# simonsobs/Pixell.jl

Measured on AMD Instinct MI355X. Metric: Mpix/s CAR bilinear reproject (Float64) + % HBM roofline, 1/2/4/8 MI355X, higher is better.
Workload: dtype f64

## Files before the change

### include/pixell_hip.h

```cpp
#ifndef PIXELL_HIP_H
#define PIXELL_HIP_H

#include <stddef.h>
#include <stdint.h>

#ifdef __cplusplus
extern "C" {
#endif

#define PXL_VERSION 100

typedef struct pxl_car_wcs {
    double cdelt[2];
    double crpix[2];
    double crval[2];
    double unit;
} pxl_car_wcs;

#define PXL_OK         0
#define PXL_EINVAL   (-22)
#define PXL_ENOMEM   (-12)
#define PXL_EHIP     (-5)
#define PXL_ENODEV   (-19)

// ... 40 lines not shown
                        double* ra, double* dec, void* stream);
int pxl_posmap_tan_f64(const pxl_car_wcs* wcs, const int64_t shape[2], int64_t row0, int64_t nrows,
                       double* ra, double* dec, void* stream);

typedef struct pxl_reproject_plan pxl_reproject_plan;

int pxl_reproject_plan_create(const pxl_car_wcs* wcs_in, const int64_t shape_in[3],
                              int64_t src_row0, int64_t src_nrows,
                              const pxl_car_wcs* wcs_out, const int64_t shape_out[2],
                              int64_t dst_row0, int64_t dst_nrows,
                              pxl_reproject_plan** plan);
int pxl_reproject_execute(pxl_reproject_plan* plan, const double* src, double* dst, void* stream);
int pxl_reproject_build_tables(pxl_reproject_plan* plan, void* stream);
int pxl_reproject_execute_rows(pxl_reproject_plan* plan, const double* src, double* dst,
                               int64_t r0, int64_t nr, void* stream);
int pxl_reproject_execute_f32(pxl_reproject_plan* plan, const float* src, float* dst, void* stream);
int pxl_reproject_execute_rows_f32(pxl_reproject_plan* plan, const float* src, float* dst,
                                   int64_t r0, int64_t nr, void* stream);
int pxl_reproject_plan_src_rows(const pxl_reproject_plan* plan, int64_t* lo, int64_t* hi);
int pxl_reproject_plan_rows_covered(const pxl_reproject_plan* plan, int64_t have_lo, int64_t have_hi,
                                    int64_t* lo, int64_t* hi);
int pxl_reproject_plan_set_variant(pxl_reproject_plan* plan, int variant);
int pxl_reproject_plan_destroy(pxl_reproject_plan* plan);

typedef struct pxl_halo_xfer {
    int32_t peer;
    int32_t reserved;
    int64_t row0;
    int64_t nrows;
} pxl_halo_xfer;
// ... 127 lines not shown
```

### pixell.jl_amd/_lib.py

```python
import ctypes as C
import os

_HERE = os.path.dirname(os.path.abspath(__file__))
LIB_PATH = os.environ.get("PXL_LIB_PATH", os.path.join(_HERE, "libpixell_hip.so"))

WRAP_NONE, WRAP_REWIND, WRAP_UNWIND = 0, 1, 2
FORM_RECIP, FORM_DIV, FORM_RECIP_AV = 0, 1, 2


class PixellHipError(RuntimeError):

    def __init__(self, code, message):
        super().__init__("libpixell_hip error %d: %s" % (code, message))
        self.code = code


class CarWCSStruct(C.Structure):
    _fields_ = [("cdelt", C.c_double * 2), ("crpix", C.c_double * 2), ("crval", C.c_double * 2),
                ("unit", C.c_double)]


_P = C.c_void_p
_I64 = C.c_int64
_WP = C.POINTER(CarWCSStruct)
# ... 10 lines not shown
    "pxl_pix2sky_car_soa_f64": (C.c_int, [_WP, _I64, _P, _P, _P, _P, C.c_int, _P]),
    "pxl_sky2pix_car_f64": (C.c_int, [_WP, _SHP, _I64, _P, _P, C.c_int, C.c_int, _P]),
    "pxl_sky2pix_car_soa_f64": (C.c_int, [_WP, _SHP, _I64, _P, _P, _P, _P, C.c_int, C.c_int, _P]),
    "pxl_posmap_car_f64": (C.c_int, [_WP, _SHP, _I64, _I64, _P, _P, C.c_int, _P]),
    "pxl_pixareamap_car_f64": (C.c_int, [_WP, _SHP, _I64, _I64, _P, _P]),
    "pxl_distance_transform_car_f64": (C.c_int, [_WP, _SHP, _P, _P, _P]),
    "pxl_sky2pix_tan_f64": (C.c_int, [_WP, _I64, _P, _P, _P, _P, _P]),
    "pxl_pix2sky_tan_f64": (C.c_int, [_WP, _I64, _P, _P, _P, _P, _P]),
    "pxl_posmap_tan_f64": (C.c_int, [_WP, _SHP, _I64, _I64, _P, _P, _P]),
    "pxl_reproject_plan_create": (C.c_int, [_WP, _SHP, _I64, _I64, _WP, _SHP, _I64, _I64, C.POINTER(_P)]),
    "pxl_reproject_execute": (C.c_int, [_P, _P, _P, _P]),
    "pxl_reproject_build_tables": (C.c_int, [_P, _P]),
    "pxl_reproject_execute_rows": (C.c_int, [_P, _P, _P, _I64, _I64, _P]),
    "pxl_reproject_execute_f32": (C.c_int, [_P, _P, _P, _P]),
    "pxl_reproject_execute_rows_f32": (C.c_int, [_P, _P, _P, _I64, _I64, _P]),
    "pxl_reproject_plan_src_rows": (C.c_int, [_P, C.POINTER(_I64), C.POINTER(_I64)]),
    "pxl_reproject_plan_rows_covered": (C.c_int, [_P, _I64, _I64, C.POINTER(_I64), C.POINTER(_I64)]),
    "pxl_reproject_plan_set_variant": (C.c_int, [_P, C.c_int]),
    "pxl_reproject_plan_destroy": (C.c_int, [_P]),
    "pxl_reproject_sharded_step_f64": (C.c_int, [_P, _P, _P, _I64, _I64, _P, C.c_int, _P, C.c_int, _P, _P]),
    "pxl_reproject_sharded_step_f32": (C.c_int, [_P, _P, _P, _I64, _I64, _P, C.c_int, _P, C.c_int, _P, _P]),
    "pxl_comm_unique_id": (C.c_int, [_P]),
    "pxl_comm_init_rank": (C.c_int, [_P, C.c_int, C.c_int, C.POINTER(_P)]),
    "pxl_comm_destroy": (C.c_int, [_P]),
    "pxl_comm_backend": (C.c_char_p, []),
    "pxl_reproject_car_bilinear_f64": (C.c_int, [_WP, _SHP, _P, _WP, _SHP, _P, _P]),
    "pxl_reproject_generic_bilinear_f64": (C.c_int, [_WP, C.c_int, _SHP, _P, _WP, C.c_int, _SHP, _P, _P]),
    "pxl_reproject_generic_last_tiles": (C.c_int, [C.POINTER(_I64), C.POINTER(_I64), _P]),
    "pxl_generic_plan_create": (C.c_int, [_WP, C.c_int, _SHP, _WP, C.c_int, _SHP, _P, C.POINTER(_P)]),
    "pxl_generic_plan_execute": (C.c_int, [_P, _I64, _P, _P, _P]),
# ... 89 lines not shown
```

### pixell.jl_amd/csrc/pxl_kernels.hip

```cpp
#include <hip/hip_runtime.h>

#include <algorithm>
#include <mutex>
#include <vector>
#include <cmath>
#include <cstdarg>
#include <cstdio>
#include <cstring>
#include <new>
#include <type_traits>

#include "pxl_device.h"

using namespace pxl;

static thread_local char g_err[512] = "";

static int fail(int code, const char* fmt, ...) {
    va_list ap;
    va_start(ap, fmt);
    vsnprintf(g_err, sizeof(g_err), fmt, ap);
    va_end(ap);
    return code;
}
// ... 72 lines not shown
static constexpr SlotRule kSlot32 = {256, 8.0, 4};
static int64_t seg_for(const SlotRule& r, int pairs, double sx) {
    double span = ceil((double)(r.cw * pairs) * sx) + r.slack;
    return ((int64_t)span + (r.align - 1)) & ~(r.align - 1);
}
static bool stageable(const SlotRule& r, int64_t sg, bool periodic, int64_t nx, double sy) {
    return (sg <= PXL_MAXCH * r.cw) && !(periodic && sg > nx) && sy <= 3.0;
}

struct pxl_reproject_plan {
    pxl_car_wcs win, wout;
    int64_t nx, ny, nc, src_row0, src_nrows;
    int64_t nxo, nyo, dst_row0, dst_nrows;
    int periodic;
    int device;
    Tables tab;
    void* table_mem;
    int32_t* h_yj0;
    int variant;
    int pairs;
    int pairs_dma;
    int seg_dma;
    int pairs_dma32;
    int seg_dma32;
    bool dma32_ok;
    int dypos;
    int rh;
    int rh32;
    int seg;
    int dxpos;
    int ns, pf;
    int nt;
    double* zero_page;
    bool staged_ok;
    bool vec_load;
    bool tables_built;
    hipStream_t comm_stream;
    hipEvent_t ev_ready, ev_halo;
    int64_t cov_have_lo, cov_have_hi, cov_lo, cov_hi;
};

struct DeviceState {
    hipMemPool_t pool;
    unsigned int* last_exact;
    int64_t generic_tiles;
};
static std::mutex g_dev_mu;
static DeviceState g_dev[64] = {};
static DeviceState* device_state() {
    int dev = 0;
    if (hipGetDevice(&dev) != hipSuccess || dev < 0 || dev >= 64) return nullptr;
// ... 171 lines not shown
    if (items < (int64_t)min_per_front * fronts) fronts = 1;
    int64_t per = (items + fronts - 1) / fronts;
    if (cap > 0 && per * fronts > cap) { fronts = 1; per = items; }
    return {fronts, per};
}

static int check_rows(const char* who, const int64_t shape[2], int64_t row0, int64_t nrows) {
    if (!shape || shape[0] < 1 || shape[1] < 1) return fail(PXL_EINVAL, "%s: bad shape", who);
    if (row0 < 0 || nrows < 0 || row0 + nrows > shape[1])
        return fail(PXL_EINVAL, "%s: rows [%lld, %lld) outside the map (ny=%lld)", who, (long long)row0,
                    (long long)(row0 + nrows), (long long)shape[1]);
    return PXL_OK;
}

template <class T>
static int reproject_rows_impl(pxl_reproject_plan* pl, const T* src, T* dst, int64_t r0, int64_t nr, void* stream) {
    if (!pl) return fail(PXL_EINVAL, "execute: null plan");
    if (r0 < 0 || nr < 0 || r0 + nr > pl->dst_nrows) return fail(PXL_EINVAL, "execute: rows outside the dst window");
    if (nr == 0) return PXL_OK;
    if (!dst || (!src && pl->src_nrows > 0)) return fail(PXL_EINVAL, "execute: null src/dst");
    if (!pl->tables_built) return fail(PXL_EINVAL, "execute_rows: tables not built");
    hipStream_t st = (hipStream_t)stream;
    constexpr bool f32 = std::is_same<T, float>::value;

    ReprojParams p;
    memset(&p, 0, sizeof(p));
    p.src = src; p.dst = dst;
    p.xi0 = pl->tab.xi0; p.xfx = pl->tab.xfx; p.yj0 = pl->tab.yj0; p.yfy = pl->tab.yfy;
    p.nx = pl->nx; p.ny = pl->ny; p.src_row0 = pl->src_row0; p.src_nrows = pl->src_nrows;
    p.nxo = pl->nxo; p.dst_row0 = pl->dst_row0; p.dst_nrows = pl->dst_nrows;
    p.r0 = r0; p.nr = nr; p.nc = (int32_t)pl->nc; p.periodic = pl->periodic;

    const bool aligned = (((uintptr_t)src & 15) == 0);
    bool staged = f32 ? (pl->dma32_ok && aligned) : pl->staged_ok;
    if (pl->variant == 1) staged = false;
    if (!staged) {
        int64_t work = ((pl->nxo + 1) / 2) * nr;
        dim3 g(stream_grid(work, 256), (unsigned)pl->nc);
        hipLaunchKernelGGL((k_reproject_gather<T>), g, dim3(256), 0, st, p);
        return check_launch("k_reproject_gather");
    }

    const bool vec = f32 ? true : (pl->vec_load && aligned);
    const bool use_dma = f32 ? true : (vec && pl->variant != 2);
    const int pairs = f32 ? pl->pairs_dma32 : (use_dma ? pl->pairs_dma : pl->pairs);
    const int cw = f32 ? kSlot32.cw : kSlot64.cw;
    const int TW = cw * pairs;
    p.seg = f32 ? pl->seg_dma32 : (use_dma ? pl->seg_dma : pl->seg);
    p.dxpos = pl->dxpos; p.dypos = pl->dypos;
    p.ntx = (int32_t)((pl->nxo + TW - 1) / TW);
    int rh = f32 ? pl->rh32 : pl->rh;
    while (rh > 4 && (int64_t)p.ntx * ((nr + rh - 1) / rh) * pl->nc < PXL_MIN_TILES) rh >>= 1;
    p.rh = rh;
    p.nty = (int32_t)((nr + rh - 1) / rh);
    p.ntiles = (int64_t)p.ntx * p.nty * pl->nc;
    p.tiles_per_xcd = (p.ntiles + 7) / 8;
    const int64_t nblocks = 8 * p.tiles_per_xcd;
    if (nblocks > 0x7fffffffLL) return fail(PXL_EINVAL, "execute: too many tiles (%lld)", (long long)nblocks);
    dim3 grid((unsigned)nblocks), block(64);
    if (use_dma) {
        const size_t esz = sizeof(T);
        p.ns = pl->ns; p.pf = pl->pf; p.zero_page = pl->zero_page;
        p.nt = pl->nt != 0;
        while ((size_t)p.ns * p.seg * esz > PXL_RING_BYTES && p.ns > 4) p.ns >>= 1;
        size_t dma_lds = (size_t)p.ns * (size_t)p.seg * esz;
        const int nch = (p.seg + cw - 1) / cw;
        return launch_reproject_dma_t<T>(pairs, nch, grid, dma_lds, st, p);
    }
    size_t lds_bytes = (size_t)PXL_NS * (size_t)pl->seg * sizeof(double);
// ... 48 lines not shown
        const ncclDataType_t dt = std::is_same<T, float>::value ? ncclFloat32 : ncclFloat64;
        ncclResult_t r = nc.GroupStart();
        for (int i = 0; i < nsends && r == ncclSuccess; ++i)
            for (int64_t c = 0; c < pl->nc && r == ncclSuccess; ++c)
                r = nc.Send((const char*)src + ((c * pl->src_nrows + (sends[i].row0 - lo)) * pl->nx) * esz,
                            (size_t)(sends[i].nrows * pl->nx), dt, sends[i].peer, (ncclComm_t)comm, pl->comm_stream);
        for (int i = 0; i < nrecvs && r == ncclSuccess; ++i)
            for (int64_t c = 0; c < pl->nc && r == ncclSuccess; ++c)
                r = nc.Recv((char*)src + ((c * pl->src_nrows + (recvs[i].row0 - lo)) * pl->nx) * esz,
                            (size_t)(recvs[i].nrows * pl->nx), dt, recvs[i].peer, (ncclComm_t)comm, pl->comm_stream);
        const ncclResult_t rend = nc.GroupEnd();
        if (r == ncclSuccess) r = rend;
        if (r != ncclSuccess) return fail(PXL_EHIP, "sharded_step: RCCL send/recv failed: %s", nc.GetErrorString(r));
        HIP_TRY(hipEventRecord(pl->ev_halo, pl->comm_stream));
    }
    rc = pxl_reproject_build_tables(pl, stream);
    if (rc) return rc;
    int64_t i_lo = 0, i_hi = pl->dst_nrows;
    if (exchange) {
        if (pl->cov_have_lo != own_row0 || pl->cov_have_hi != own_row0 + own_nrows || pl->cov_hi < pl->cov_lo) {
            rc = pxl_reproject_plan_rows_covered(pl, own_row0, own_row0 + own_nrows, &pl->cov_lo, &pl->cov_hi);
            if (rc) return rc;
            pl->cov_have_lo = own_row0; pl->cov_have_hi = own_row0 + own_nrows;
        }
        i_lo = pl->cov_lo; i_hi = pl->cov_hi;
    }
    if (i_hi > i_lo) {
        rc = reproject_rows_impl<T>(pl, src, dst, i_lo, i_hi - i_lo, stream);
        if (rc) return rc;
    }
    if (exchange) {
        HIP_TRY(hipStreamWaitEvent(st, pl->ev_halo, 0));
        if (i_hi > i_lo) {
            if (i_lo > 0) { rc = reproject_rows_impl<T>(pl, src, dst, 0, i_lo, stream); if (rc) return rc; }
            if (i_hi < pl->dst_nrows) rc = reproject_rows_impl<T>(pl, src, dst, i_hi, pl->dst_nrows - i_hi, stream);
        } else {
            rc = reproject_rows_impl<T>(pl, src, dst, 0, pl->dst_nrows, stream);
        }
    }
    return rc;
}

static unsigned int* last_exact_word(int64_t total_tiles = -1, int64_t* total_out = nullptr) {
    DeviceState* d = device_state();
    if (!d) return nullptr;
    std::lock_guard<std::mutex> lock(g_dev_mu);
    if (!d->last_exact) {
        if (hipMalloc((void**)&d->last_exact, 64) != hipSuccess || hipMemset(d->last_exact, 0, 64) != hipSuccess) {
            (void)hipGetLastError(); d->last_exact = nullptr; return nullptr;
        }
// ... 439 lines not shown
        return fail(PXL_EINVAL, "plan_create: axis too long (source RA axis <= 4e8, others <= 1e9 pixels)");
    if (src_row0 < 0 || src_nrows < 0 || src_row0 + src_nrows > shape_in[1])
        return fail(PXL_EINVAL, "plan_create: source window outside the map");
    if (dst_row0 < 0 || dst_nrows < 0 || dst_row0 + dst_nrows > shape_out[1])
        return fail(PXL_EINVAL, "plan_create: destination window outside the map");

    pxl_reproject_plan* pl = new (std::nothrow) pxl_reproject_plan();
    if (!pl) return fail(PXL_ENOMEM, "plan_create: host allocation failed");
    pl->cov_lo = 0; pl->cov_hi = -1;
    pl->win = *wcs_in; pl->wout = *wcs_out;
    pl->nx = shape_in[0]; pl->ny = shape_in[1]; pl->nc = shape_in[2];
    pl->src_row0 = src_row0; pl->src_nrows = src_nrows;
    pl->nxo = shape_out[0]; pl->nyo = shape_out[1];
    pl->dst_row0 = dst_row0; pl->dst_nrows = dst_nrows;
    pl->periodic = car_periodic(wcs_in, pl->nx);
    pl->tables_built = false;

    hipError_t e = hipGetDevice(&pl->device);
    if (e != hipSuccess) { delete pl; return fail(PXL_ENODEV, "hipGetDevice: %s", hipGetErrorString(e)); }

    const size_t nyo = (size_t)pl->nyo, off_zero = table_layout(nullptr, pl->nxo, pl->nyo).bytes, total = off_zero + 64;
    e = hipMalloc(&pl->table_mem, total);
    if (e != hipSuccess) { delete pl; return fail(PXL_ENOMEM, "plan_create: hipMalloc(%zu): %s", total, hipGetErrorString(e)); }
    char* base = (char*)pl->table_mem;
    e = hipMemset(base + off_zero, 0, 64);
    if (e != hipSuccess) { (void)hipFree(pl->table_mem); delete pl; return fail(PXL_EHIP, "plan_create: hipMemset: %s", hipGetErrorString(e)); }
    pl->zero_page = (double*)(base + off_zero);
    pl->tab = table_layout(base, pl->nxo, pl->nyo);

    pl->h_yj0 = new (std::nothrow) int32_t[nyo];
    if (!pl->h_yj0) { (void)hipFree(pl->table_mem); delete pl; return fail(PXL_ENOMEM, "plan_create: host allocation failed"); }
    CarAffine co = car_affine(pl->wout);
    Sky2Pix si = sky2pix_setup(pl->win, pl->nx, pl->ny, 1, PXL_FORM_DIV);
    for (int64_t j = 0; j < pl->nyo; ++j) {
        double fr;
        split_cell(s2p_y(si, p2s_dec(co, (double)(j + 1))), &pl->h_yj0[j], &fr);
    }

    double sx = fabs((pl->wout.cdelt[0] * pl->wout.unit) / (pl->win.cdelt[0] * pl->win.unit));
    pl->dxpos = ((pl->wout.cdelt[0] * pl->wout.unit) / (pl->win.cdelt[0] * pl->win.unit)) > 0 ? 1 : 0;
    pl->dypos = ((pl->wout.cdelt[1] * pl->wout.unit) / (pl->win.cdelt[1] * pl->win.unit)) > 0 ? 1 : 0;
    double sy = fabs((pl->wout.cdelt[1] * pl->wout.unit) / (pl->win.cdelt[1] * pl->win.unit));
    pl->rh = env_int("PXL_REPROJECT_RH", sy >= 1.5 ? 4 : (sy > 0.3 ? 16 : 8));
    if (pl->rh < 1) pl->rh = 1;
    if (pl->rh > 64) pl->rh = 64;
    pl->rh32 = env_int("PXL_REPROJECT_RH", 32);
    if (pl->rh32 < 1) pl->rh32 = 1;
    if (pl->rh32 > 64) pl->rh32 = 64;
    pl->ns = env_int("PXL_REPROJECT_NS", (double)pl->nx * (double)pl->ny * (double)pl->nc * 8.0 <= 128.0 * 1048576.0 ? 4 : 8);
    if (pl->ns < 4) pl->ns = 4;
    while (pl->ns & (pl->ns - 1)) pl->ns &= pl->ns - 1;
// ... 32 lines not shown

int pxl_reproject_plan_set_variant(pxl_reproject_plan* pl, int variant) {
    if (!pl || variant < 0 || variant > 2) return fail(PXL_EINVAL, "set_variant: bad argument");
    pl->variant = variant;
    return PXL_OK;
}

int pxl_reproject_plan_destroy(pxl_reproject_plan* pl) {
    if (!pl) return PXL_OK;
    if (pl->comm_stream) {
        (void)hipStreamSynchronize(pl->comm_stream);
        (void)hipEventDestroy(pl->ev_ready);
        (void)hipEventDestroy(pl->ev_halo);
        (void)hipStreamDestroy(pl->comm_stream);
    }
    if (pl->table_mem) (void)hipFree(pl->table_mem);
    delete[] pl->h_yj0;
    delete pl;
    return PXL_OK;
}

int pxl_reproject_build_tables(pxl_reproject_plan* pl, void* stream) {
    if (!pl) return fail(PXL_EINVAL, "build_tables: null plan");
    launch_build_tables(pl->win, pl->nx, pl->ny, pl->wout, pl->nxo, pl->nyo, pl->tab, (hipStream_t)stream);
    int rc = check_launch("k_build_tables");
    if (rc == PXL_OK) pl->tables_built = true;
    return rc;
}

int pxl_reproject_execute_rows(pxl_reproject_plan* pl, const double* src, double* dst, int64_t r0, int64_t nr,
                               void* stream) {
    return reproject_rows_impl(pl, src, dst, r0, nr, stream);
}

int pxl_reproject_execute_rows_f32(pxl_reproject_plan* pl, const float* src, float* dst, int64_t r0, int64_t nr,
                                   void* stream) {
    return reproject_rows_impl(pl, src, dst, r0, nr, stream);
}

int pxl_reproject_execute(pxl_reproject_plan* pl, const double* src, double* dst, void* stream) {
    int rc = pxl_reproject_build_tables(pl, stream);
    if (rc) return rc;
    return pxl_reproject_execute_rows(pl, src, dst, 0, pl->dst_nrows, stream);
}

int pxl_reproject_execute_f32(pxl_reproject_plan* pl, const float* src, float* dst, void* stream) {
    int rc = pxl_reproject_build_tables(pl, stream);
    if (rc) return rc;
    return pxl_reproject_execute_rows_f32(pl, src, dst, 0, pl->dst_nrows, stream);
}

int pxl_reproject_plan_src_rows(const pxl_reproject_plan* pl, int64_t* lo, int64_t* hi) {
    if (!pl || !lo || !hi) return fail(PXL_EINVAL, "plan_src_rows: null argument");
    int64_t l = INT64_MAX, h = INT64_MIN;
    for (int64_t r = 0; r < pl->dst_nrows; ++r) {
        int64_t j0 = pl->h_yj0[pl->dst_row0 + r];
        for (int64_t j = j0; j <= j0 + 1; ++j)
            if (j >= 1 && j <= pl->ny) { if (j - 1 < l) l = j - 1; if (j > h) h = j; }
    }
    if (l > h) { l = 0; h = 0; }
    *lo = l; *hi = h;
    return PXL_OK;
}
// ... 480 lines not shown
```

### pixell.jl_amd/csrc/pxl_reproject.h

```cpp
#pragma once

__global__ __launch_bounds__(256) void k_build_tables(CarAffine out, Sky2Pix in, int64_t nxo, int64_t nyo,
                                                      int32_t* __restrict__ xi0, double* __restrict__ xfx,
                                                      int32_t* __restrict__ yj0, double* __restrict__ yfy) {
    int64_t stride = (int64_t)gridDim.x * blockDim.x;
    for (int64_t k = (int64_t)blockIdx.x * blockDim.x + threadIdx.x; k < nxo + nyo; k += stride) {
        if (k < nxo) {
            double a = p2s_ra(out, (double)(k + 1));
            split_cell(s2p_x(in, a), &xi0[k], &xfx[k]);
        } else {
            int64_t j = k - nxo;
            double d = p2s_dec(out, (double)(j + 1));
            split_cell(s2p_y(in, d), &yj0[j], &yfy[j]);
        }
    }
}

struct ReprojParams {
    const void* src;
    void* dst;
    const int32_t* xi0; const double* xfx;
    const int32_t* yj0; const double* yfy;
    int64_t nx, ny, src_row0, src_nrows;
    int64_t nxo, dst_row0, dst_nrows;
    int64_t r0, nr;
    int32_t nc, periodic;
    int32_t rh;
    int32_t seg;
    int32_t dxpos;
    int32_t dypos;
    int32_t ntx, nty;
    int64_t ntiles, tiles_per_xcd;
    int32_t ns, pf;
    int32_t nt;
    const double* zero_page;
};

__device__ inline int64_t xcd_tile(int64_t b, int64_t tiles_per_xcd) {
    return (b & 7) * tiles_per_xcd + (b >> 3);
}

template <typename T>
__global__ __launch_bounds__(256) void k_reproject_gather(ReprojParams p) {
    const int64_t npair = (p.nxo + 1) / 2;
    const int64_t total = npair * p.nr;
    const int c = blockIdx.y;
    SrcViewT<T> m{(const T*)p.src + (int64_t)c * p.nx * p.src_nrows, p.nx, p.ny, p.src_row0, p.src_nrows, p.periodic};
    T* dplane = (T*)p.dst + (int64_t)c * p.nxo * p.dst_nrows;
    int64_t stride = (int64_t)gridDim.x * blockDim.x;
    for (int64_t t = (int64_t)blockIdx.x * blockDim.x + threadIdx.x; t < total; t += stride) {
        int64_t rr = t / npair;
        int64_t i = (t - rr * npair) * 2;
        int64_t r = p.r0 + rr;
        int64_t j0 = p.yj0[p.dst_row0 + r];
        double fy = p.yfy[p.dst_row0 + r];
        int64_t o = r * p.nxo + i;
        dplane[o] = (T)bilerp_cells(m, p.xi0[i], p.xfx[i], j0, fy);
        if (i + 1 < p.nxo) dplane[o + 1] = (T)bilerp_cells(m, p.xi0[i + 1], p.xfx[i + 1], j0, fy);
    }
}

#define PXL_NS 4
#define PXL_MAXCH 5

template <bool VEC>
__device__ inline void load_row_regs(const ReprojParams& p, const double* plane, int64_t j, int64_t cbase0,
                                     int lane, double2 (&regs)[PXL_MAXCH]) {
    int64_t jr = j - 1 - p.src_row0;
    const bool row_ok = (j >= 1) && (j <= p.ny) && (jr >= 0) && (jr < p.src_nrows);
    const double* rowp = plane + (row_ok ? jr : 0) * p.nx;
#pragma unroll
    for (int ch = 0; ch < PXL_MAXCH; ++ch) {
        int k = ch * 128 + 2 * lane;
// ... 37 lines not shown
    const int lane = threadIdx.x;
    constexpr int TW = 128 * PAIRS;

    const int64_t t = xcd_tile(blockIdx.x, p.tiles_per_xcd);
    if (t >= p.ntiles) return;
    const int tx = (int)(t % p.ntx);
    const int64_t trest = t / p.ntx;
    const int ty = (int)(trest % p.nty);
    const int c = (int)(trest / p.nty);

    const double* splane = (const double*)p.src + (int64_t)c * p.nx * p.src_nrows;
    double* dplane = (double*)p.dst + (int64_t)c * p.nxo * p.dst_nrows;

    const int64_t c0 = (int64_t)tx * TW;
    const int64_t clast = (c0 + TW < p.nxo ? c0 + TW : p.nxo) - 1;
    const int64_t rb = p.r0 + (int64_t)ty * p.rh;
    const int64_t re = (rb + p.rh < p.r0 + p.nr) ? rb + p.rh : p.r0 + p.nr;

    const int64_t a = p.dxpos ? p.xi0[c0] : p.xi0[clast];
    const int64_t ua = a - 1;
    const int64_t cbase0 = ua & ~(int64_t)1;
    int dloc[PAIRS][2];
    double fx[PAIRS][2];
    bool act[PAIRS][2];
    bool fits = true;
#pragma unroll
    for (int q = 0; q < PAIRS; ++q) {
#pragma unroll
        for (int e = 0; e < 2; ++e) {
            int64_t col = c0 + q * 128 + 2 * lane + e;
            act[q][e] = col < p.nxo;
            int64_t i0 = act[q][e] ? p.xi0[col] : a;
            fx[q][e] = act[q][e] ? p.xfx[col] : 0.0;
            int64_t d = i0 - a;
            if (p.periodic) { d %= p.nx; if (d < 0) d += p.nx; }
            d += ua - cbase0;
            if (d < 0 || d + 1 >= p.seg) fits = false;
            dloc[q][e] = (int)d;
        }
    }
    const bool vec_store = ((p.nxo & 1) == 0) && (((uintptr_t)p.dst & 15) == 0);

    if (!__all(fits)) {
        SrcView m{splane, p.nx, p.ny, p.src_row0, p.src_nrows, p.periodic};
        for (int64_t r = rb; r < re; ++r) {
            int64_t j0 = p.yj0[p.dst_row0 + r];
            double fy = p.yfy[p.dst_row0 + r];
#pragma unroll
            for (int q = 0; q < PAIRS; ++q)
#pragma unroll
                for (int e = 0; e < 2; ++e) {
                    int64_t col = c0 + q * 128 + 2 * lane + e;
                    if (act[q][e]) dplane[r * p.nxo + col] = bilerp_cells(m, p.xi0[col], fx[q][e], j0, fy);
                }
        }
        return;
    }

    int64_t tag0 = INT64_MIN, tag1 = INT64_MIN, tag2 = INT64_MIN, tag3 = INT64_MIN;
    auto resident = [&](int64_t j) -> bool {
        int s = (int)(j & 3);
        int64_t tg = (s == 0) ? tag0 : (s == 1) ? tag1 : (s == 2) ? tag2 : tag3;
        return tg == j;
    };
    auto settag = [&](int64_t j) {
        int s = (int)(j & 3);
        if (s == 0) tag0 = j; else if (s == 1) tag1 = j; else if (s == 2) tag2 = j; else tag3 = j;
    };

    int my_j0 = 0;
    double my_fy = 0.0;
    if (rb + lane < re) { my_j0 = p.yj0[p.dst_row0 + rb + lane]; my_fy = p.yfy[p.dst_row0 + rb + lane]; }
    auto row_j0 = [&](int64_t r) -> int64_t { return (int64_t)__builtin_amdgcn_readlane(my_j0, (int)(r - rb)); };
    auto row_fy = [&](int64_t r) -> double {
        int lo = __builtin_amdgcn_readlane(__double2loint(my_fy), (int)(r - rb));
        int hi = __builtin_amdgcn_readlane(__double2hiint(my_fy), (int)(r - rb));
        return __hiloint2double(hi, lo);
    };

    double2 ra_[PXL_MAXCH], rb_[PXL_MAXCH];
    {
        int64_t j0 = row_j0(rb);
        load_row_regs<VEC>(p, splane, j0, cbase0, lane, ra_);
        load_row_regs<VEC>(p, splane, j0 + 1, cbase0, lane, rb_);
        store_row_lds(p, lds + (j0 & 3) * p.seg, lane, ra_);
        store_row_lds(p, lds + ((j0 + 1) & 3) * p.seg, lane, rb_);
        settag(j0); settag(j0 + 1);
// ... 46 lines not shown
```

### pixell.jl_amd/csrc/pxl_reproject_dma.h

```cpp
#pragma once

template <int N>
__device__ __forceinline__ void wait_vm() {
    asm volatile("s_waitcnt vmcnt(%0)" ::"n"(N) : "memory");
}

__device__ __forceinline__ void wait_vm_upto(int k) {
    if (k < 8) {
        if (k < 4) {
            if (k < 2) { if (k < 1) wait_vm<0>(); else wait_vm<1>(); }
            else       { if (k < 3) wait_vm<2>(); else wait_vm<3>(); }
        } else {
            if (k < 6) { if (k < 5) wait_vm<4>(); else wait_vm<5>(); }
            else       { if (k < 7) wait_vm<6>(); else wait_vm<7>(); }
        }
    } else if (k < 16) {
        if (k < 12) {
            if (k < 10) { if (k < 9) wait_vm<8>(); else wait_vm<9>(); }
            else        { if (k < 11) wait_vm<10>(); else wait_vm<11>(); }
        } else {
            if (k < 14) { if (k < 13) wait_vm<12>(); else wait_vm<13>(); }
            else        { if (k < 15) wait_vm<14>(); else wait_vm<15>(); }
        }
    } else {
// ... 20 lines not shown
    constexpr int CW = 64 * EPL;
    constexpr int TW = CW * PAIRS;

    const int64_t t = xcd_tile(blockIdx.x, p.tiles_per_xcd);
    if (t >= p.ntiles) return;
    const int tx = (int)(t % p.ntx);
    const int64_t trest = t / p.ntx;
    const int ty = (int)(trest % p.nty);
    const int c = (int)(trest / p.nty);

    const T* splane = (const T*)p.src + (int64_t)c * p.nx * p.src_nrows;
    T* dplane = (T*)p.dst + (int64_t)c * p.nxo * p.dst_nrows;

    const int64_t c0 = (int64_t)tx * TW;
    const int64_t clast = (c0 + TW < p.nxo ? c0 + TW : p.nxo) - 1;
    const int64_t rb = p.r0 + (int64_t)ty * p.rh;
    const int64_t re = (rb + p.rh < p.r0 + p.nr) ? rb + p.rh : p.r0 + p.nr;
    const int nrows = (int)(re - rb);

    const int64_t a = p.dxpos ? p.xi0[c0] : p.xi0[clast];
    const int64_t ua = a - 1;
    const int64_t cbase0 = ua - (((ua % EPL) + EPL) % EPL);
    int dloc[PAIRS][EPL];
    double fx[PAIRS][EPL];
    bool act[PAIRS][EPL];
    bool fits = true;
#pragma unroll
    for (int q = 0; q < PAIRS; ++q) {
#pragma unroll
        for (int e = 0; e < EPL; ++e) {
            int64_t col = c0 + q * CW + EPL * lane + e;
            act[q][e] = col < p.nxo;
            int64_t i0 = act[q][e] ? p.xi0[col] : a;
            fx[q][e] = act[q][e] ? p.xfx[col] : 0.0;
            int64_t d = i0 - a;
            if (p.periodic) { d %= p.nx; if (d < 0) d += p.nx; }
            d += ua - cbase0;
            if (d < 0 || d + 1 >= p.seg) fits = false;
            dloc[q][e] = (int)d;
        }
    }

    int my_j0 = 0;
    double my_fy = 0.0;
    if (lane < nrows) { my_j0 = p.yj0[p.dst_row0 + rb + lane]; my_fy = p.yfy[p.dst_row0 + rb + lane]; }
    const int dir = p.dypos ? 1 : -1;
    const int my_t0 = p.dypos ? my_j0 : -(my_j0 + 1);
    const double my_wa = p.dypos ? 1 - my_fy : my_fy;
    const double my_wb = p.dypos ? my_fy : 1 - my_fy;
    {
        int nxt = __shfl_down(my_t0, 1, 64);
        bool mono = (lane + 1 >= nrows) || (nxt >= my_t0);
        if (!mono) fits = false;
    }

    if (!__all(fits)) {
        SrcViewT<T> m{splane, p.nx, p.ny, p.src_row0, p.src_nrows, p.periodic};
        for (int64_t r = rb; r < re; ++r) {
            int64_t j0 = p.yj0[p.dst_row0 + r];
            double fy = p.yfy[p.dst_row0 + r];
#pragma unroll
            for (int q = 0; q < PAIRS; ++q)
#pragma unroll
                for (int e = 0; e < EPL; ++e) {
                    int64_t col = c0 + q * CW + EPL * lane + e;
                    if (act[q][e]) dplane[r * p.nxo + col] = (T)bilerp_cells(m, p.xi0[col], fx[q][e], j0, fy);
                }
        }
        return;
    }

    uint32_t voff[NCH];
#pragma unroll
    for (int ch = 0; ch < NCH; ++ch) {
        int64_t u = cbase0 + ch * CW + EPL * lane;
        bool ok = true;
        if (p.periodic) { u %= p.nx; if (u < 0) u += p.nx; }
        else ok = (u >= 0) && (u < p.nx);
        voff[ch] = ok ? (uint32_t)(u * (int64_t)sizeof(T)) : 0xFFFFFFFFu;
    }

// ... 134 lines not shown
```

### pixell.jl_amd/ops.py

```python
import ctypes as C

import torch

from . import _lib, placement
from ._lib import FORM_DIV, FORM_RECIP, FORM_RECIP_AV, WRAP_NONE, WRAP_REWIND, WRAP_UNWIND
from .enmap import Enmap, _geom
from .wcs import (AbstractCARWCS, Gnomonic, pix2sky_scalar, pix2sky_tan_scalar, sky2pix_scalar,
                  sky2pix_tan_scalar)


def _stream(t: torch.Tensor):
    return C.c_void_p(torch.cuda.current_stream(t.device).cuda_stream)


def _dev_f64(t: torch.Tensor, what: str) -> torch.Tensor:
    if not isinstance(t, torch.Tensor):
        raise TypeError("%s must be a torch tensor" % what)
    if not t.is_cuda:
        raise RuntimeError("%s must live on the GPU: the MI355X path has no CPU fallback "
                           "(CPU arrays stay with the reference implementation)" % what)
    if t.dtype != torch.float64:
        raise TypeError("%s must be float64" % what)
    if not t.is_contiguous():
        raise ValueError("%s must be contiguous" % what)
# ... 323 lines not shown
        with torch.cuda.device(self.device):
            _lib.check(fn(self._h, _ptr(src), _ptr(dst), _stream(dst)))
        return dst

    def build_tables(self):
        with torch.cuda.device(self.device):
            s = C.c_void_p(torch.cuda.current_stream(self.device).cuda_stream)
            _lib.check(_lib.load().pxl_reproject_build_tables(self._h, s))

    def execute_rows(self, src, dst, r0, nr):
        src, dst = self._check(src, dst)
        lib = _lib.load()
        fn = lib.pxl_reproject_execute_rows_f32 if src.dtype == torch.float32 else lib.pxl_reproject_execute_rows
        with torch.cuda.device(self.device):
            _lib.check(fn(self._h, _ptr(src), _ptr(dst), r0, nr, _stream(dst)))
        return dst

    def close(self):
        if getattr(self, "_h", None) is not None and self._h.value:
            _lib.load().pxl_reproject_plan_destroy(self._h)
            self._h = C.c_void_p()

    def __del__(self):
        try:
            self.close()
        except Exception:
            pass


def _check_order(order):
# ... 524 lines not shown
```

### pixell.jl_amd/sharding.py

```python
import numpy as np
import torch
import torch.distributed as dist

from .wcs import TWOPI


def strip_bounds(n: int, world: int, rank: int):
    return (n * rank) // world, (n * (rank + 1)) // world


def _np_jl_mod(x, y: float):
    r = np.fmod(x, y)
    zero = r == 0.0
    flip = (r > 0.0) != (y > 0.0)
    r = np.where(flip & ~zero, r + y, r)
    return np.where(zero, np.copysign(0.0, y), r)


def _np_rewind(a, period: float, ref: float):
    half = period / 2
    return (ref + _np_jl_mod((a - ref) + half, period)) - half


def host_row_cells(shape_in, wcs_in, shape_out, wcs_out):
# ... 226 lines not shown
            self._xfers = (_lib.xfer_arr(self.sends), _lib.xfer_arr(self.recvs))
        if comm_ptr is None and (self.sends or self.recvs):
            comm_ptr = self.rccl_comm_ptr()
        fn = lib.pxl_reproject_sharded_step_f32 if src.dtype == torch.float32 else lib.pxl_reproject_sharded_step_f64
        own_lo, own_hi = self.own[self.rank]
        with torch.cuda.device(self.device):
            s = C.c_void_p(torch.cuda.current_stream(self.device).cuda_stream)
            _lib.check(fn(self.plan._h, C.c_void_p(src.data_ptr()), C.c_void_p(dst.data_ptr()), own_lo, own_hi - own_lo,
                          C.cast(self._xfers[0], C.c_void_p), len(self.sends), C.cast(self._xfers[1], C.c_void_p), len(self.recvs),
                          C.c_void_p(comm_ptr or 0), s))
        return dst

    def step(self, src: torch.Tensor, dst: torch.Tensor, events=None):
        nrows = self.dst_window[1]
        if self.world == 1 or (not self.sends and not self.recvs):
            self.plan.build_tables()
            if events:
                events[0].record()
            self.plan.execute_rows(src, dst, 0, nrows)
            if events:
                events[1].record()
            return dst
        if self._staging is None:
            self._staging = self.make_staging(src, self.group)
        works = self.start_halo_exchange(src, self._staging, self.group)
        self.plan.build_tables()
        i_lo, i_hi = self.interior
        if i_hi > i_lo:
            if events:
                events[0].record()
            self.plan.execute_rows(src, dst, i_lo, i_hi - i_lo)
            if events:
                events[1].record()
        self.finish_halo_exchange(src, self._staging, works)
        if i_hi > i_lo:
            if i_lo > 0:
                self.plan.execute_rows(src, dst, 0, i_lo)
            if i_hi < nrows:
                self.plan.execute_rows(src, dst, i_hi, nrows - i_hi)
        else:
            if events:
                events[0].record()
            self.plan.execute_rows(src, dst, 0, nrows)
            if events:
                events[1].record()
        return dst
```

Measured before the change: 387,600.

## Compute bilinear coordinates inline and merge boundary row ranges into one launch

Drops the precomputed per-column and per-row coordinate tables and their build kernel. The reproject kernels now evaluate the CAR affine and sky2pix mapping on the fly from plan parameters. Separately, the two halo boundary row bands are executed in a single launch via a second row range instead of two launches. This removes a table-build kernel per step and the table memory reads, at the cost of extra floating-point math (including divisions) per tile and per element in the gather path.

```diff
diff --git a/include/pixell_hip.h b/include/pixell_hip.h
--- a/include/pixell_hip.h
+++ b/include/pixell_hip.h
@@ -78,6 +78,10 @@
 int pxl_reproject_build_tables(pxl_reproject_plan* plan, void* stream);
 int pxl_reproject_execute_rows(pxl_reproject_plan* plan, const double* src, double* dst,
                                int64_t r0, int64_t nr, void* stream);
+int pxl_reproject_execute_rows2(pxl_reproject_plan* plan, const double* src, double* dst,
+                                int64_t r0, int64_t nr, int64_t r1, int64_t nr1, void* stream);
+int pxl_reproject_execute_rows2_f32(pxl_reproject_plan* plan, const float* src, float* dst,
+                                    int64_t r0, int64_t nr, int64_t r1, int64_t nr1, void* stream);
 int pxl_reproject_execute_f32(pxl_reproject_plan* plan, const float* src, float* dst, void* stream);
 int pxl_reproject_execute_rows_f32(pxl_reproject_plan* plan, const float* src, float* dst,
                                    int64_t r0, int64_t nr, void* stream);
diff --git a/pixell.jl_amd/_lib.py b/pixell.jl_amd/_lib.py
--- a/pixell.jl_amd/_lib.py
+++ b/pixell.jl_amd/_lib.py
@@ -48,6 +48,8 @@
     "pxl_reproject_execute_rows": (C.c_int, [_P, _P, _P, _I64, _I64, _P]),
     "pxl_reproject_execute_f32": (C.c_int, [_P, _P, _P, _P]),
     "pxl_reproject_execute_rows_f32": (C.c_int, [_P, _P, _P, _I64, _I64, _P]),
+    "pxl_reproject_execute_rows2": (C.c_int, [_P, _P, _P, _I64, _I64, _I64, _I64, _P]),
+    "pxl_reproject_execute_rows2_f32": (C.c_int, [_P, _P, _P, _I64, _I64, _I64, _I64, _P]),
     "pxl_reproject_plan_src_rows": (C.c_int, [_P, C.POINTER(_I64), C.POINTER(_I64)]),
     "pxl_reproject_plan_rows_covered": (C.c_int, [_P, _I64, _I64, C.POINTER(_I64), C.POINTER(_I64)]),
     "pxl_reproject_plan_set_variant": (C.c_int, [_P, C.c_int]),
diff --git a/pixell.jl_amd/csrc/pxl_kernels.hip b/pixell.jl_amd/csrc/pxl_kernels.hip
--- a/pixell.jl_amd/csrc/pxl_kernels.hip
+++ b/pixell.jl_amd/csrc/pxl_kernels.hip
@@ -110,8 +110,8 @@
     int64_t nxo, nyo, dst_row0, dst_nrows;
     int periodic;
     int device;
-    Tables tab;
-    void* table_mem;
+    CarAffine out;
+    Sky2Pix in;
     int32_t* h_yj0;
     int variant;
     int pairs;
@@ -130,7 +130,6 @@
     double* zero_page;
     bool staged_ok;
     bool vec_load;
-    bool tables_built;
     hipStream_t comm_stream;
     hipEvent_t ev_ready, ev_halo;
     int64_t cov_have_lo, cov_have_hi, cov_lo, cov_hi;
@@ -332,28 +331,31 @@
 }
 
 template <class T>
-static int reproject_rows_impl(pxl_reproject_plan* pl, const T* src, T* dst, int64_t r0, int64_t nr, void* stream) {
+static int reproject_rows_impl(pxl_reproject_plan* pl, const T* src, T* dst, int64_t r0, int64_t nr, void* stream,
+                               int64_t r1 = 0, int64_t nr1 = 0) {
     if (!pl) return fail(PXL_EINVAL, "execute: null plan");
     if (r0 < 0 || nr < 0 || r0 + nr > pl->dst_nrows) return fail(PXL_EINVAL, "execute: rows outside the dst window");
+    if (r1 < 0 || nr1 < 0 || r1 + nr1 > pl->dst_nrows) return fail(PXL_EINVAL, "execute: rows outside the dst window");
+    if (nr == 0) { r0 = r1; nr = nr1; r1 = 0; nr1 = 0; }
     if (nr == 0) return PXL_OK;
+    if (nr1 > 0 && r0 < r1 + nr1 && r1 < r0 + nr) return fail(PXL_EINVAL, "execute: the two row ranges overlap");
     if (!dst || (!src && pl->src_nrows > 0)) return fail(PXL_EINVAL, "execute: null src/dst");
-    if (!pl->tables_built) return fail(PXL_EINVAL, "execute_rows: tables not built");
     hipStream_t st = (hipStream_t)stream;
     constexpr bool f32 = std::is_same<T, float>::value;
 
     ReprojParams p;
     memset(&p, 0, sizeof(p));
     p.src = src; p.dst = dst;
-    p.xi0 = pl->tab.xi0; p.xfx = pl->tab.xfx; p.yj0 = pl->tab.yj0; p.yfy = pl->tab.yfy;
+    p.out = pl->out; p.in = pl->in;
     p.nx = pl->nx; p.ny = pl->ny; p.src_row0 = pl->src_row0; p.src_nrows = pl->src_nrows;
     p.nxo = pl->nxo; p.dst_row0 = pl->dst_row0; p.dst_nrows = pl->dst_nrows;
-    p.r0 = r0; p.nr = nr; p.nc = (int32_t)pl->nc; p.periodic = pl->periodic;
+    p.r0 = r0; p.nr = nr; p.r1 = r1; p.nr1 = nr1; p.nc = (int32_t)pl->nc; p.periodic = pl->periodic;
 
     const bool aligned = (((uintptr_t)src & 15) == 0);
     bool staged = f32 ? (pl->dma32_ok && aligned) : pl->staged_ok;
     if (pl->variant == 1) staged = false;
     if (!staged) {
-        int64_t work = ((pl->nxo + 1) / 2) * nr;
+        int64_t work = ((pl->nxo + 1) / 2) * (nr + nr1);
         dim3 g(stream_grid(work, 256), (unsigned)pl->nc);
         hipLaunchKernelGGL((k_reproject_gather<T>), g, dim3(256), 0, st, p);
         return check_launch("k_reproject_gather");
@@ -368,9 +370,10 @@
     p.dxpos = pl->dxpos; p.dypos = pl->dypos;
     p.ntx = (int32_t)((pl->nxo + TW - 1) / TW);
     int rh = f32 ? pl->rh32 : pl->rh;
-    while (rh > 4 && (int64_t)p.ntx * ((nr + rh - 1) / rh) * pl->nc < PXL_MIN_TILES) rh >>= 1;
+    while (rh > 4 && (int64_t)p.ntx * ((nr + rh - 1) / rh + (nr1 + rh - 1) / rh) * pl->nc < PXL_MIN_TILES) rh >>= 1;
     p.rh = rh;
-    p.nty = (int32_t)((nr + rh - 1) / rh);
+    p.nty0 = (int32_t)((nr + rh - 1) / rh);
+    p.nty = p.nty0 + (int32_t)((nr1 + rh - 1) / rh);
     p.ntiles = (int64_t)p.ntx * p.nty * pl->nc;
     p.tiles_per_xcd = (p.ntiles + 7) / 8;
     const int64_t nblocks = 8 * p.tiles_per_xcd;
@@ -449,8 +452,6 @@
         if (r != ncclSuccess) return fail(PXL_EHIP, "sharded_step: RCCL send/recv failed: %s", nc.GetErrorString(r));
         HIP_TRY(hipEventRecord(pl->ev_halo, pl->comm_stream));
     }
-    rc = pxl_reproject_build_tables(pl, stream);
-    if (rc) return rc;
     int64_t i_lo = 0, i_hi = pl->dst_nrows;
     if (exchange) {
         if (pl->cov_have_lo != own_row0 || pl->cov_have_hi != own_row0 + own_nrows || pl->cov_hi < pl->cov_lo) {
@@ -467,8 +468,7 @@
     if (exchange) {
         HIP_TRY(hipStreamWaitEvent(st, pl->ev_halo, 0));
         if (i_hi > i_lo) {
-            if (i_lo > 0) { rc = reproject_rows_impl<T>(pl, src, dst, 0, i_lo, stream); if (rc) return rc; }
-            if (i_hi < pl->dst_nrows) rc = reproject_rows_impl<T>(pl, src, dst, i_hi, pl->dst_nrows - i_hi, stream);
+            rc = reproject_rows_impl<T>(pl, src, dst, 0, i_lo, stream, i_hi, pl->dst_nrows - i_hi);
         } else {
             rc = reproject_rows_impl<T>(pl, src, dst, 0, pl->dst_nrows, stream);
         }
@@ -938,27 +938,22 @@
     pl->nxo = shape_out[0]; pl->nyo = shape_out[1];
     pl->dst_row0 = dst_row0; pl->dst_nrows = dst_nrows;
     pl->periodic = car_periodic(wcs_in, pl->nx);
-    pl->tables_built = false;
 
     hipError_t e = hipGetDevice(&pl->device);
     if (e != hipSuccess) { delete pl; return fail(PXL_ENODEV, "hipGetDevice: %s", hipGetErrorString(e)); }
 
-    const size_t nyo = (size_t)pl->nyo, off_zero = table_layout(nullptr, pl->nxo, pl->nyo).bytes, total = off_zero + 64;
-    e = hipMalloc(&pl->table_mem, total);
-    if (e != hipSuccess) { delete pl; return fail(PXL_ENOMEM, "plan_create: hipMalloc(%zu): %s", total, hipGetErrorString(e)); }
-    char* base = (char*)pl->table_mem;
-    e = hipMemset(base + off_zero, 0, 64);
-    if (e != hipSuccess) { (void)hipFree(pl->table_mem); delete pl; return fail(PXL_EHIP, "plan_create: hipMemset: %s", hipGetErrorString(e)); }
-    pl->zero_page = (double*)(base + off_zero);
-    pl->tab = table_layout(base, pl->nxo, pl->nyo);
-
-    pl->h_yj0 = new (std::nothrow) int32_t[nyo];
-    if (!pl->h_yj0) { (void)hipFree(pl->table_mem); delete pl; return fail(PXL_ENOMEM, "plan_create: host allocation failed"); }
-    CarAffine co = car_affine(pl->wout);
-    Sky2Pix si = sky2pix_setup(pl->win, pl->nx, pl->ny, 1, PXL_FORM_DIV);
+    e = hipMalloc((void**)&pl->zero_page, 64);
+    if (e != hipSuccess) { delete pl; return fail(PXL_ENOMEM, "plan_create: hipMalloc(64): %s", hipGetErrorString(e)); }
+    e = hipMemset(pl->zero_page, 0, 64);
+    if (e != hipSuccess) { (void)hipFree(pl->zero_page); delete pl; return fail(PXL_EHIP, "plan_create: hipMemset: %s", hipGetErrorString(e)); }
+    pl->out = car_affine(pl->wout);
+    pl->in = sky2pix_setup(pl->win, pl->nx, pl->ny, 1, PXL_FORM_DIV);
+
+    pl->h_yj0 = new (std::nothrow) int32_t[(size_t)pl->nyo];
+    if (!pl->h_yj0) { (void)hipFree(pl->zero_page); delete pl; return fail(PXL_ENOMEM, "plan_create: host allocation failed"); }
     for (int64_t j = 0; j < pl->nyo; ++j) {
         double fr;
-        split_cell(s2p_y(si, p2s_dec(co, (double)(j + 1))), &pl->h_yj0[j], &fr);
+        split_cell(s2p_y(pl->in, p2s_dec(pl->out, (double)(j + 1))), &pl->h_yj0[j], &fr);
     }
 
     double sx = fabs((pl->wout.cdelt[0] * pl->wout.unit) / (pl->win.cdelt[0] * pl->win.unit));
@@ -1021,18 +1016,16 @@
         (void)hipEventDestroy(pl->ev_halo);
         (void)hipStreamDestroy(pl->comm_stream);
     }
-    if (pl->table_mem) (void)hipFree(pl->table_mem);
+    if (pl->zero_page) (void)hipFree(pl->zero_page);
     delete[] pl->h_yj0;
     delete pl;
     return PXL_OK;
 }
 
 int pxl_reproject_build_tables(pxl_reproject_plan* pl, void* stream) {
+    (void)stream;
     if (!pl) return fail(PXL_EINVAL, "build_tables: null plan");
-    launch_build_tables(pl->win, pl->nx, pl->ny, pl->wout, pl->nxo, pl->nyo, pl->tab, (hipStream_t)stream);
-    int rc = check_launch("k_build_tables");
-    if (rc == PXL_OK) pl->tables_built = true;
-    return rc;
+    return PXL_OK;
 }
 
 int pxl_reproject_execute_rows(pxl_reproject_plan* pl, const double* src, double* dst, int64_t r0, int64_t nr,
@@ -1045,15 +1038,23 @@
     return reproject_rows_impl(pl, src, dst, r0, nr, stream);
 }
 
+int pxl_reproject_execute_rows2(pxl_reproject_plan* pl, const double* src, double* dst, int64_t r0, int64_t nr,
+                                int64_t r1, int64_t nr1, void* stream) {
+    return reproject_rows_impl(pl, src, dst, r0, nr, stream, r1, nr1);
+}
+
+int pxl_reproject_execute_rows2_f32(pxl_reproject_plan* pl, const float* src, float* dst, int64_t r0, int64_t nr,
+                                    int64_t r1, int64_t nr1, void* stream) {
+    return reproject_rows_impl(pl, src, dst, r0, nr, stream, r1, nr1);
+}
+
 int pxl_reproject_execute(pxl_reproject_plan* pl, const double* src, double* dst, void* stream) {
-    int rc = pxl_reproject_build_tables(pl, stream);
-    if (rc) return rc;
+    if (!pl) return fail(PXL_EINVAL, "execute: null plan");
     return pxl_reproject_execute_rows(pl, src, dst, 0, pl->dst_nrows, stream);
 }
 
 int pxl_reproject_execute_f32(pxl_reproject_plan* pl, const float* src, float* dst, void* stream) {
-    int rc = pxl_reproject_build_tables(pl, stream);
-    if (rc) return rc;
+    if (!pl) return fail(PXL_EINVAL, "execute: null plan");
     return pxl_reproject_execute_rows_f32(pl, src, dst, 0, pl->dst_nrows, stream);
 }
 
diff --git a/pixell.jl_amd/csrc/pxl_reproject.h b/pixell.jl_amd/csrc/pxl_reproject.h
--- a/pixell.jl_amd/csrc/pxl_reproject.h
+++ b/pixell.jl_amd/csrc/pxl_reproject.h
@@ -19,17 +19,19 @@
 struct ReprojParams {
     const void* src;
     void* dst;
-    const int32_t* xi0; const double* xfx;
-    const int32_t* yj0; const double* yfy;
+    CarAffine out;
+    Sky2Pix in;
     int64_t nx, ny, src_row0, src_nrows;
     int64_t nxo, dst_row0, dst_nrows;
     int64_t r0, nr;
+    int64_t r1, nr1;
     int32_t nc, periodic;
     int32_t rh;
     int32_t seg;
     int32_t dxpos;
     int32_t dypos;
     int32_t ntx, nty;
+    int32_t nty0;
     int64_t ntiles, tiles_per_xcd;
     int32_t ns, pf;
     int32_t nt;
@@ -40,10 +42,30 @@
     return (b & 7) * tiles_per_xcd + (b >> 3);
 }
 
+__device__ inline void col_entry(const ReprojParams& p, int64_t ic, int32_t* cell, double* frac) {
+    split_cell(s2p_x(p.in, p2s_ra(p.out, (double)(ic + 1))), cell, frac);
+}
+__device__ inline void row_entry(const ReprojParams& p, int64_t j, int32_t* cell, double* frac) {
+    split_cell(s2p_y(p.in, p2s_dec(p.out, (double)(j + 1))), cell, frac);
+}
+__device__ inline int64_t col_cell_uniform(const ReprojParams& p, int64_t ic) {
+    int32_t cell; double frac;
+    col_entry(p, ic, &cell, &frac);
+    return (int64_t)__builtin_amdgcn_readfirstlane(cell);
+}
+
+__device__ inline void tile_rows(const ReprojParams& p, int ty, int64_t* rb, int64_t* re) {
+    const bool second = ty >= p.nty0;
+    const int64_t lo = second ? p.r1 : p.r0, hi = lo + (second ? p.nr1 : p.nr);
+    const int64_t b = lo + (int64_t)(second ? ty - p.nty0 : ty) * p.rh;
+    *rb = b;
+    *re = (b + p.rh < hi) ? b + p.rh : hi;
+}
+
 template <typename T>
 __global__ __launch_bounds__(256) void k_reproject_gather(ReprojParams p) {
     const int64_t npair = (p.nxo + 1) / 2;
-    const int64_t total = npair * p.nr;
+    const int64_t total = npair * (p.nr + p.nr1);
     const int c = blockIdx.y;
     SrcViewT<T> m{(const T*)p.src + (int64_t)c * p.nx * p.src_nrows, p.nx, p.ny, p.src_row0, p.src_nrows, p.periodic};
     T* dplane = (T*)p.dst + (int64_t)c * p.nxo * p.dst_nrows;
@@ -51,12 +73,17 @@
     for (int64_t t = (int64_t)blockIdx.x * blockDim.x + threadIdx.x; t < total; t += stride) {
         int64_t rr = t / npair;
         int64_t i = (t - rr * npair) * 2;
-        int64_t r = p.r0 + rr;
-        int64_t j0 = p.yj0[p.dst_row0 + r];
-        double fy = p.yfy[p.dst_row0 + r];
+        int64_t r = rr < p.nr ? p.r0 + rr : p.r1 + (rr - p.nr);
+        int32_t j0, i0;
+        double fy, fx;
+        row_entry(p, p.dst_row0 + r, &j0, &fy);
         int64_t o = r * p.nxo + i;
-        dplane[o] = (T)bilerp_cells(m, p.xi0[i], p.xfx[i], j0, fy);
-        if (i + 1 < p.nxo) dplane[o + 1] = (T)bilerp_cells(m, p.xi0[i + 1], p.xfx[i + 1], j0, fy);
+        col_entry(p, i, &i0, &fx);
+        dplane[o] = (T)bilerp_cells(m, i0, fx, j0, fy);
+        if (i + 1 < p.nxo) {
+            col_entry(p, i + 1, &i0, &fx);
+            dplane[o + 1] = (T)bilerp_cells(m, i0, fx, j0, fy);
+        }
     }
 }
 
@@ -124,13 +151,14 @@
 
     const int64_t c0 = (int64_t)tx * TW;
     const int64_t clast = (c0 + TW < p.nxo ? c0 + TW : p.nxo) - 1;
-    const int64_t rb = p.r0 + (int64_t)ty * p.rh;
-    const int64_t re = (rb + p.rh < p.r0 + p.nr) ? rb + p.rh : p.r0 + p.nr;
-
-    const int64_t a = p.dxpos ? p.xi0[c0] : p.xi0[clast];
+    int64_t rb, re;
+    tile_rows(p, ty, &rb, &re);
+
+    const int64_t a = col_cell_uniform(p, p.dxpos ? c0 : clast);
     const int64_t ua = a - 1;
     const int64_t cbase0 = ua & ~(int64_t)1;
     int dloc[PAIRS][2];
+    int32_t ci[PAIRS][2];
     double fx[PAIRS][2];
     bool act[PAIRS][2];
     bool fits = true;
@@ -140,8 +168,9 @@
         for (int e = 0; e < 2; ++e) {
             int64_t col = c0 + q * 128 + 2 * lane + e;
             act[q][e] = col < p.nxo;
-            int64_t i0 = act[q][e] ? p.xi0[col] : a;
-            fx[q][e] = act[q][e] ? p.xfx[col] : 0.0;
+            col_entry(p, col, &ci[q][e], &fx[q][e]);
+            int64_t i0 = act[q][e] ? (int64_t)ci[q][e] : a;
+            fx[q][e] = act[q][e] ? fx[q][e] : 0.0;
             int64_t d = i0 - a;
             if (p.periodic) { d %= p.nx; if (d < 0) d += p.nx; }
             d += ua - cbase0;
@@ -154,14 +183,15 @@
     if (!__all(fits)) {
         SrcView m{splane, p.nx, p.ny, p.src_row0, p.src_nrows, p.periodic};
         for (int64_t r = rb; r < re; ++r) {
-            int64_t j0 = p.yj0[p.dst_row0 + r];
-            double fy = p.yfy[p.dst_row0 + r];
+            int32_t j0;
+            double fy;
+            row_entry(p, p.dst_row0 + r, &j0, &fy);
 #pragma unroll
             for (int q = 0; q < PAIRS; ++q)
 #pragma unroll
                 for (int e = 0; e < 2; ++e) {
                     int64_t col = c0 + q * 128 + 2 * lane + e;
-                    if (act[q][e]) dplane[r * p.nxo + col] = bilerp_cells(m, p.xi0[col], fx[q][e], j0, fy);
+                    if (act[q][e]) dplane[r * p.nxo + col] = bilerp_cells(m, ci[q][e], fx[q][e], j0, fy);
                 }
         }
         return;
@@ -180,7 +210,7 @@
 
     int my_j0 = 0;
     double my_fy = 0.0;
-    if (rb + lane < re) { my_j0 = p.yj0[p.dst_row0 + rb + lane]; my_fy = p.yfy[p.dst_row0 + rb + lane]; }
+    if (rb + lane < re) row_entry(p, p.dst_row0 + rb + lane, &my_j0, &my_fy);
     auto row_j0 = [&](int64_t r) -> int64_t { return (int64_t)__builtin_amdgcn_readlane(my_j0, (int)(r - rb)); };
     auto row_fy = [&](int64_t r) -> double {
         int lo = __builtin_amdgcn_readlane(__double2loint(my_fy), (int)(r - rb));
diff --git a/pixell.jl_amd/csrc/pxl_reproject_dma.h b/pixell.jl_amd/csrc/pxl_reproject_dma.h
--- a/pixell.jl_amd/csrc/pxl_reproject_dma.h
+++ b/pixell.jl_amd/csrc/pxl_reproject_dma.h
@@ -58,14 +58,15 @@
 
     const int64_t c0 = (int64_t)tx * TW;
     const int64_t clast = (c0 + TW < p.nxo ? c0 + TW : p.nxo) - 1;
-    const int64_t rb = p.r0 + (int64_t)ty * p.rh;
-    const int64_t re = (rb + p.rh < p.r0 + p.nr) ? rb + p.rh : p.r0 + p.nr;
+    int64_t rb, re;
+    tile_rows(p, ty, &rb, &re);
     const int nrows = (int)(re - rb);
 
-    const int64_t a = p.dxpos ? p.xi0[c0] : p.xi0[clast];
+    const int64_t a = col_cell_uniform(p, p.dxpos ? c0 : clast);
     const int64_t ua = a - 1;
     const int64_t cbase0 = ua - (((ua % EPL) + EPL) % EPL);
     int dloc[PAIRS][EPL];
+    int32_t ci[PAIRS][EPL];
     double fx[PAIRS][EPL];
     bool act[PAIRS][EPL];
     bool fits = true;
@@ -75,8 +76,9 @@
         for (int e = 0; e < EPL; ++e) {
             int64_t col = c0 + q * CW + EPL * lane + e;
             act[q][e] = col < p.nxo;
-            int64_t i0 = act[q][e] ? p.xi0[col] : a;
-            fx[q][e] = act[q][e] ? p.xfx[col] : 0.0;
+            col_entry(p, col, &ci[q][e], &fx[q][e]);
+            int64_t i0 = act[q][e] ? (int64_t)ci[q][e] : a;
+            fx[q][e] = act[q][e] ? fx[q][e] : 0.0;
             int64_t d = i0 - a;
             if (p.periodic) { d %= p.nx; if (d < 0) d += p.nx; }
             d += ua - cbase0;
@@ -87,7 +89,7 @@
 
     int my_j0 = 0;
     double my_fy = 0.0;
-    if (lane < nrows) { my_j0 = p.yj0[p.dst_row0 + rb + lane]; my_fy = p.yfy[p.dst_row0 + rb + lane]; }
+    if (lane < nrows) row_entry(p, p.dst_row0 + rb + lane, &my_j0, &my_fy);
     const int dir = p.dypos ? 1 : -1;
     const int my_t0 = p.dypos ? my_j0 : -(my_j0 + 1);
     const double my_wa = p.dypos ? 1 - my_fy : my_fy;
@@ -101,14 +103,15 @@
     if (!__all(fits)) {
         SrcViewT<T> m{splane, p.nx, p.ny, p.src_row0, p.src_nrows, p.periodic};
         for (int64_t r = rb; r < re; ++r) {
-            int64_t j0 = p.yj0[p.dst_row0 + r];
-            double fy = p.yfy[p.dst_row0 + r];
+            int32_t j0;
+            double fy;
+            row_entry(p, p.dst_row0 + r, &j0, &fy);
 #pragma unroll
             for (int q = 0; q < PAIRS; ++q)
 #pragma unroll
                 for (int e = 0; e < EPL; ++e) {
                     int64_t col = c0 + q * CW + EPL * lane + e;
-                    if (act[q][e]) dplane[r * p.nxo + col] = (T)bilerp_cells(m, p.xi0[col], fx[q][e], j0, fy);
+                    if (act[q][e]) dplane[r * p.nxo + col] = (T)bilerp_cells(m, ci[q][e], fx[q][e], j0, fy);
                 }
         }
         return;
diff --git a/pixell.jl_amd/ops.py b/pixell.jl_amd/ops.py
--- a/pixell.jl_amd/ops.py
+++ b/pixell.jl_amd/ops.py
@@ -361,6 +361,14 @@
         fn = lib.pxl_reproject_execute_rows_f32 if src.dtype == torch.float32 else lib.pxl_reproject_execute_rows
         with torch.cuda.device(self.device):
             _lib.check(fn(self._h, _ptr(src), _ptr(dst), r0, nr, _stream(dst)))
+        return dst
+
+    def execute_rows2(self, src, dst, r0, nr, r1, nr1):
+        src, dst = self._check(src, dst)
+        lib = _lib.load()
+        fn = lib.pxl_reproject_execute_rows2_f32 if src.dtype == torch.float32 else lib.pxl_reproject_execute_rows2
+        with torch.cuda.device(self.device):
+            _lib.check(fn(self._h, _ptr(src), _ptr(dst), r0, nr, r1, nr1, _stream(dst)))
         return dst
 
     def close(self):
diff --git a/pixell.jl_amd/sharding.py b/pixell.jl_amd/sharding.py
--- a/pixell.jl_amd/sharding.py
+++ b/pixell.jl_amd/sharding.py
@@ -264,7 +264,6 @@
     def step(self, src: torch.Tensor, dst: torch.Tensor, events=None):
         nrows = self.dst_window[1]
         if self.world == 1 or (not self.sends and not self.recvs):
-            self.plan.build_tables()
             if events:
                 events[0].record()
             self.plan.execute_rows(src, dst, 0, nrows)
@@ -274,7 +273,6 @@
         if self._staging is None:
             self._staging = self.make_staging(src, self.group)
         works = self.start_halo_exchange(src, self._staging, self.group)
-        self.plan.build_tables()
         i_lo, i_hi = self.interior
         if i_hi > i_lo:
             if events:
@@ -284,10 +282,8 @@
                 events[1].record()
         self.finish_halo_exchange(src, self._staging, works)
         if i_hi > i_lo:
-            if i_lo > 0:
-                self.plan.execute_rows(src, dst, 0, i_lo)
-            if i_hi < nrows:
-                self.plan.execute_rows(src, dst, i_hi, nrows - i_hi)
+            if i_lo > 0 or i_hi < nrows:
+                self.plan.execute_rows2(src, dst, 0, i_lo, i_hi, nrows - i_hi)
         else:
             if events:
                 events[0].record()
```

Result: no change. 389,000, median of 4 (+0.4%).
